# JVBSouza/descriptools

Measured on AMD Instinct MI355X. Metric: Mcells/s full descriptor chain, higher is better.
Workload: dtype f32; 1 GPU; 16384x16384 synthetic tilted-integer-fBm DEM per GPU, full chain (d8, flowacc, river mask, flowhand/HAND with fused GFI + ln(hl/H), fused slope+TI+MTI, downslope), device-resident; global_dem=16384x16384, river_threshold_cells=524288

## Files before the change

### descriptools_amd/_lib.py

```python
import ctypes as C
import os

import numpy as np

_HERE = os.path.dirname(os.path.abspath(__file__))
_SO = os.path.join(_HERE, "libdescriptools_hip.so")
_lib = None

c_f32p = C.POINTER(C.c_float)
c_f64p = C.POINTER(C.c_double)
c_u8p = C.POINTER(C.c_uint8)
c_u16p = C.POINTER(C.c_uint16)
c_i8p = C.POINTER(C.c_int8)
c_i32p = C.POINTER(C.c_int32)
c_i64p = C.POINTER(C.c_int64)
i64, f64, u32, ci = C.c_int64, C.c_double, C.c_uint32, C.c_int
vp = C.c_void_p

_SIGS = {
    "dt_last_error": (C.c_char_p, []),
    "dt_version": (C.c_char_p, []),
    "dt_device_count": (ci, []),
    "dt_set_flow_impl": (ci, [ci]),
    "dt_debug_set": (ci, [ci, ci]),
# ... 76 lines not shown
    "dt_gfi_area": (ci, [c_f32p, c_i64p, i64, f64, f64, f64, ci, c_f32p]),
    "dt_gfi": (ci, [c_f32p, c_i64p, c_i64p, i64, f64, f64, f64, c_f32p]),
    "dt_lnhlh": (ci, [c_f32p, c_i64p, i64, f64, f64, f64, c_f32p]),
    "dt_downslope": (ci, [c_f32p, c_u8p, i64, i64, f64, f64, ci, c_f32p]),
    "dt_slope_f64": (ci, [c_f64p, i64, i64, f64, c_f32p]),
    "dt_hand_f64": (ci, [c_f64p, c_i64p, i64, c_f64p]),
    "dt_downslope_f64": (ci, [c_f64p, c_u8p, i64, i64, f64, f64, ci, c_f32p]),
    "dt_gfi_f64h": (ci, [c_f64p, c_i64p, c_i64p, i64, f64, f64, f64, ci, c_f32p]),
    "dt_d8_f64": (ci, [c_f64p, i64, i64, f64, c_u8p, c_f32p]),
    "dt_confusion_multi": (ci, [c_f64p, c_i8p, i64, f64, c_f64p, ci, ci, c_i64p]),
    "dt_threshold_hist": (ci, [c_f64p, c_i8p, i64, f64, c_f64p, ci, ci, c_i64p]),
    "dt_synth_dem": (ci, [u32, i64, i64, i64, i64, i64, i64, ci, c_f32p]),
    "dt_dev_malloc": (ci, [vp, i64, C.POINTER(vp)]),
    "dt_dev_free": (ci, [vp, vp]),
    "dt_dev_h2d": (ci, [vp, vp, vp, i64]),
    "dt_dev_d2h": (ci, [vp, vp, vp, i64]),
    "dt_dev_d2h_async": (ci, [vp, vp, vp, i64]),
    "dt_dev_synth_dem": (ci, [vp, u32, i64, i64, i64, i64, i64, i64, ci, vp]),
    "dt_dev_slope_d8": (ci, [vp, vp, i64, i64, f64, vp, vp, vp]),
    "dt_dev_slope_twi": (ci, [vp, vp, vp, i64, i64, f64, f64, vp, vp, vp, vp]),
    "dt_dev_flowacc": (ci, [vp, vp, vp, i64, i64, vp]),
    "dt_dev_flowacc_weighted": (ci, [vp, vp, vp, vp, i64, i64, ci, vp]),
    "dt_dev_stream_order": (ci, [vp, vp, vp, i64, i64, vp, vp, vp]),
    "dt_dev_drainage": (ci, [vp, vp, vp, vp, i64, i64, f64, vp, vp, vp]),
    "dt_dev_upslope_length": (ci, [vp, vp, vp, i64, i64, f64, vp]),
    "dt_dev_flowpath_upslope": (ci, [vp, vp, vp, vp, i64, i64, ci, vp, vp]),
    "dt_dev_flowpath_downstream": (ci, [vp, vp, vp, vp, vp, i64, i64, ci, vp, vp]),
    "dt_dev_carve_blend": (ci, [vp, vp, vp, vp, i64, i64, f64, vp]),
    "dt_dev_flowpath_downstream_sum": (ci, [vp, vp, vp, vp, vp, i64, i64, ci, vp]),
    "dt_dev_flowpath_upslope_longest": (ci, [vp, vp, vp, vp, i64, i64, ci, vp]),
    "dt_dev_dinf_direction": (ci, [vp, vp, vp, i64, i64, f64, vp, vp]),
    "dt_dev_dinf_accumulate": (ci, [vp, vp, vp, i64, i64, ci, ci, vp]),
    "dt_dev_dinf_accumulate_info": (ci, [vp, c_i64p]),
    "dt_dev_mfd_shares": (ci, [vp, vp, vp, i64, i64, f64, ci, vp]),
    "dt_dev_mfd_accumulate": (ci, [vp, vp, vp, i64, i64, ci, ci, vp]),
    "dt_dev_mfd_accumulate_info": (ci, [vp, c_i64p]),
    "dt_dev_mfd_route": (ci, [vp, vp, vp, vp, i64, i64, ci, ci, ci] + [vp] * 4),
    "dt_dev_dinf_route": (ci, [vp, vp, vp, vp, i64, i64, ci, ci, ci] + [vp] * 4),
    "dt_dev_cost_distance": (ci, [vp, vp, vp, i64, i64, f64, ci, ci, ci, vp, vp, vp]),
    "dt_dev_wetness_suction": (ci, [vp, vp, i64, i64, f64, f64, f64, f64, vp]),
    "dt_dev_wetness_modified_area": (ci, [vp, vp, vp, i64, i64, ci, ci, vp]),
    "dt_dev_wetness_index": (ci, [vp, vp, vp, i64, i64, f64, f64, vp]),
    "dt_dev_resample": (ci, [vp, vp, ci, i64, i64, c_f64p, ci, i64, C.c_uint64, vp, i64, i64]),
    "dt_dev_morph_reconstruct": (ci, [vp, ci, ci, ci, vp, vp, vp, f64, ci, i64, i64, ci, ci, vp, vp]),
    "dt_dev_harmonic": (ci, [vp, vp, vp, vp, i64, i64, f64, ci, vp, vp]),
    "dt_dev_inundation": (ci, [vp, vp, vp, vp, i64, i64, c_f64p, ci, vp, vp, vp, ci, ci, i64, i64, vp, vp, vp, vp, vp,
                               vp]),
    "dt_dev_terrain": (ci, [vp, vp, i64, i64, f64, ci, f64, f64, f64] + [vp] * 8),
    "dt_dev_horizon": (ci, [vp, vp, i64, i64, f64, ci, ci, f64] + [vp] * 5),
    "dt_dev_focal": (ci, [vp, vp, i64, i64, f64, ci, c_i32p, ci] + [vp] * 6),
    "dt_dev_filter_extremes": (ci, [vp, vp, i64, i64, ci] + [vp] * 5),
    "dt_dev_filter_rank": (ci, [vp, vp, i64, i64, ci, c_u16p, ci, vp]),
    "dt_dev_filter_denoise": (ci, [vp, vp, i64, i64, f64, ci, f64, ci, f64, vp]),
    "dt_dev_mrvbf": (ci, [vp, vp, i64, i64, f64, f64, ci, f64, f64, c_f64p, vp, vp]),
    "dt_dev_percentile": (ci, [vp, vp, i64, i64, ci, vp, vp]),
    "dt_dev_coarsen": (ci, [vp, vp, i64, i64, f64, c_f64p, vp, vp]),
    "dt_dev_reach_catchments": (ci, [vp, vp, vp, ci, i64, i64, vp, vp, vp, i64, vp]),
    "dt_dev_reach_channels": (ci, [vp, vp, vp, i64, i64, i64, vp, vp, vp, vp, vp]),
    "dt_dev_reach_tables": (ci, [vp, vp, vp, ci, vp, i64, i64, c_f64p, ci, i64, ci, vp, vp, vp]),
    "dt_dev_inundate": (ci, [vp, vp, vp, ci, vp, i64, i64, i64, vp]),
    "dt_dev_zonal_compact": (ci, [vp, vp, ci, i64, i64, i64, vp, vp, i64, vp]),
    "dt_dev_zonal_tables": (ci, [vp, vp, vp, ci, i64, i64, i64, f64, ci, ci, f64, vp, vp, vp, vp, vp, vp]),
    "dt_dev_zonal_counts": (ci, [vp, vp, vp, ci, i64, i64, i64, c_f64p, ci, ci, f64, vp]),
    "dt_dev_zonal_paint": (ci, [vp, vp, ci, i64, vp, i64, i64, vp, vp]),
    "dt_dev_regions_label": (ci, [vp, vp, i64, i64, ci, vp, vp]),
    "dt_dev_regions_select": (ci, [vp, vp, vp, i64, i64, ci, i64, vp]),
# ... 232 lines not shown
```

### descriptools_amd/csrc/dt_capi.hip

```cpp
#include <cmath>
#include <stdarg.h>
#include <stdlib.h>

#include <sys/mman.h>
#include <atomic>
#include <chrono>
#include <mutex>
#include <system_error>
#include <thread>
#include <utility>
#include <vector>

#include "dt_common.h"
#include "dt_kernels.h"

static thread_local char g_err[512] = "";
void dt_set_error(const char *fmt, ...) {
  va_list ap;
  va_start(ap, fmt);
  vsnprintf(g_err, sizeof(g_err), fmt, ap);
  va_end(ap);
}
extern "C" const char *dt_last_error(void) { return g_err; }
extern "C" const char *dt_version(void) { return "descriptools_hip 0.1 (gfx950)"; }
// ... 1748 lines not shown
                                                      int32_t *acc32, int8_t *river, uint8_t *kind, int32_t *ref,
                                                      int32_t *nc, int32_t *nd, float *zr, int64_t *ar) {
  return dev_flowacc_finish_fh_local_w(c, win, fdr, dem, ext_perim, threshold, acc32, 0, river, kind, ref, nc, nd, zr, ar);
}
extern "C" int dt_dev_flowacc_finish_flowhand_local_w_a64(dt_ctx *c, const dt_window *win, const uint8_t *fdr,
                                                          const float *dem, const uint64_t *ext_perim,
                                                          int64_t threshold, int64_t *acc64, int8_t *river,
                                                          uint8_t *kind, int32_t *ref, int32_t *nc, int32_t *nd,
                                                          float *zr, int64_t *ar) {
  return dev_flowacc_finish_fh_local_w(c, win, fdr, dem, ext_perim, threshold, acc64, 1, river, kind, ref, nc, nd, zr, ar);
}

static int dev_flowacc_river_flowhand_local(dt_ctx *c, const uint8_t *fdr, const float *dem, const uint8_t *nod4,
                                           int64_t H, int64_t W, int64_t threshold, int32_t *acc32, int8_t *river,
                                           const DtTwiEpilogue *twi = nullptr) {
  DT_DEV(d, c, H, W);
  DT_REQUIRE((fdr && acc32 && river) || H * W == 0, "NULL raster");
  DT_REQUIRE(!twi || H * W == 0 || dt_twi_epilogue_ok(d.w, acc32, river, twi),
             "this raster does not take the TI / MTI epilogue (dt_slope_from_d8_ok): use dt_dev_slope_twi");
  const size_t need = dt_flowacc_tiled_scratch(H, W), need2 = dt_flowhand_tiled_scratch(H, W);
  void *scr, *scr2;
  d.scratch(need, need2, &scr, &scr2);
  DT_TRY(d.rc);
  DT_TRY(dt_launch_fa_local(c->stream, d.w, fdr, scr, need, acc32, 0));
  int walked = 0;
  DT_TRY(d.done(dt_launch_fa_finish_fh_local(c->stream, d.w, fdr, dem, scr, scr2, need2, nullptr, threshold, acc32, 0,
                                             river, c->status, nod4, dt_nodata4_ld(W), twi, &walked)));
  dt_scratch_claim(c, walked ? DT_OWNER_HAND_WALK : DT_OWNER_HAND, H, W, scr2);
  return DT_OK;
}
extern "C" int dt_dev_flowacc_river_flowhand_local(dt_ctx *c, const uint8_t *fdr, const float *dem, int64_t H, int64_t W,
                                                   int64_t threshold, int32_t *acc32, int8_t *river) {
  return dev_flowacc_river_flowhand_local(c, fdr, dem, nullptr, H, W, threshold, acc32, river);
}
extern "C" int dt_dev_flowacc_river_flowhand_local_m(dt_ctx *c, const uint8_t *fdr, const float *dem,
                                                     const uint8_t *nodata4, int64_t H, int64_t W, int64_t threshold,
                                                     int32_t *acc32, int8_t *river) {
  DT_REQUIRE((dem && nodata4) || H * W == 0, "dem and the nodata mask are both required");
  return dev_flowacc_river_flowhand_local(c, fdr, dem, nodata4, H, W, threshold, acc32, river);
}
extern "C" int dt_dev_flowacc_river_flowhand_local_ms(dt_ctx *c, const uint8_t *fdr, const float *dem,
                                                      const uint8_t *nodata4, int64_t H, int64_t W, int64_t threshold,
                                                      int32_t *acc32, int8_t *river, double px, double n_top,
                                                      const float *slope, float *ti, float *mti, void *marks) {
  DT_REQUIRE((dem && nodata4 && slope && ti && mti && marks) || H * W == 0, "NULL raster");
  const DtTwiEpilogue twi{slope, ti, mti, px, n_top, marks};
  return dev_flowacc_river_flowhand_local(c, fdr, dem, nodata4, H, W, threshold, acc32, river, &twi);
}
extern "C" int dt_slope_from_d8_ok(int64_t H, int64_t W) {
  return H > 0 && W > 0 && W % 64 == 0;
}
extern "C" int64_t dt_slope_marks_bytes(int64_t H, int64_t W) {
  return (H < 0 || W < 0) ? -1 : (int64_t)dt_stencil_aux_bytes(H, W);
}
extern "C" int dt_dev_slope_twi_fix(dt_ctx *c, const float *dem, const int32_t *acc32, int64_t H, int64_t W, double px,
                                    double n_top, float *slope, float *ti, float *mti, const void *marks) {
  DT_DEV(d, c, H, W);
  DT_REQUIRE((dem && acc32 && slope && ti && mti && marks) || H * W == 0, "NULL raster");
  return d.done(dt_launch_slope_twi_fix(c->stream, d.w, dem, px, slope, acc32, n_top, ti, mti, (void *)marks));
}
extern "C" int64_t dt_nodata_mask_bytes(int64_t H, int64_t W) {
  return (H < 0 || W < 0) ? -1 : (int64_t)dt_nodata4_bytes(H, W);
}
extern "C" int dt_dev_slope_d8_m(dt_ctx *c, const float *dem, int64_t H, int64_t W, double px, uint8_t *fdr,
                                 uint8_t *nodata4) {
  DT_DEV(d, c, H, W);
// ... 1997 lines not shown
```

### descriptools_amd/csrc/dt_kernels.h

```cpp
#pragma once
#include "dt_common.h"

int dt_launch_synth_dem(hipStream_t s, uint32_t seed, int O, int64_t Hg, int64_t y0, int64_t x0,
                        int64_t h, int64_t w, int nodata_pct, float *out);
int dt_launch_stencil(hipStream_t s, const DtWin &w, const float *dem, double px, float *slope,
                      uint8_t *fdr, float *slope_rad, const void *acc, int acc64, double n_top, float *ti,
                      float *mti, void *aux = nullptr, uint8_t *nod4 = nullptr, int ldm = 0);
static inline int dt_nodata4_ld(int64_t W) { return (int)((((W + 3) / 4) + 7) & ~(int64_t)7); }
static inline size_t dt_nodata4_bytes(int64_t H, int64_t W) { return (size_t)((H + 3) / 4) * (size_t)dt_nodata4_ld(W) * 2; }
struct DtStencilAux {
  uint8_t *mark;
  uint16_t *lmask;
  size_t bytes;
};
static inline DtStencilAux dt_stencil_aux_layout(int64_t ntiles, void *aux) {
  DtStencilAux a;
  DtCarver c(aux);
  a.mark = c.take<uint8_t>((size_t)ntiles);
  a.lmask = c.take<uint16_t>((size_t)ntiles * 256);
  a.bytes = c.bytes();
  return a;
}
size_t dt_stencil_aux_bytes(int64_t H, int64_t W);
int dt_launch_d8_slope(hipStream_t s, const DtWin &w, const float *dem, double px, uint8_t *fdr, float *slope,
// ... 75 lines not shown
int dt_launch_ds_walk_seed_f64(hipStream_t s, const DtWin &w, const double *dem, int64_t n, const int32_t *ys,
                               const int32_t *xs, void *rec);
int dt_launch_confusion(hipStream_t s, const double *desc, const int8_t *flood, int64_t n,
                        double nodata, const double *th_host, int nth, int under,
                        unsigned long long *counts4);
int dt_launch_threshold_hist(hipStream_t s, const double *desc, const int8_t *flood, int64_t n, double nodata,
                             const double *th_dev, int K, int under, unsigned long long *hist);
int dt_launch_i32_to_i64(hipStream_t s, const int32_t *a, int64_t n, int64_t *b);
int dt_launch_i64_to_i32(hipStream_t s, const int64_t *a, int64_t n, int32_t *b);

size_t dt_flowacc_tiled_scratch(int64_t H, int64_t W);
int dt_launch_fa_local(hipStream_t s, const DtWin &w, const uint8_t *fdr, void *scratch, size_t scratch_bytes,
                       int32_t *acc32, int rank_level);
int dt_launch_fa_summary(hipStream_t s, const DtWin &w, void *scratch, int64_t *A, int32_t *xr, uint8_t *code);
int dt_launch_fa_finish(hipStream_t s, const DtWin &w, const uint8_t *fdr, const float *dem, void *scratch,
                        const unsigned long long *ext_perim, int64_t river_thr, void *acc, int acc64,
                        int8_t *river, int *status = nullptr);
size_t dt_flowacc_weighted_scratch(int64_t H, int64_t W);
int dt_launch_flowacc_weighted(hipStream_t s, const DtWin &w, const uint8_t *fdr, const float *dem, const double *wt,
                               int frac_bits, void *scratch, size_t scratch_bytes, double *acc, int *status);
size_t dt_flowhand_tiled_scratch(int64_t H, int64_t W);
struct DtTwiEpilogue {
  const float *slope;
  float *ti, *mti;
  double px, n_top;
  void *marks;
};
int dt_launch_fa_finish_fh_local(hipStream_t s, const DtWin &w, const uint8_t *fdr, const float *dem, void *fa_scratch,
                                 void *fh_scratch, size_t fh_bytes, const unsigned long long *ext_perim,
                                 int64_t river_thr, void *acc, int acc64, int8_t *river, int *status,
                                 const uint8_t *nod4 = nullptr, int ldm = 0, const DtTwiEpilogue *twi = nullptr,
                                 int *walked = nullptr);
bool dt_twi_epilogue_ok(const DtWin &w, const void *acc, const int8_t *river, const DtTwiEpilogue *twi);
int dt_launch_fh_local(hipStream_t s, const DtWin &w, const uint8_t *fdr, const int8_t *river, void *scratch,
                       size_t scratch_bytes);
int dt_launch_fh_summary(hipStream_t s, const DtWin &w, void *scratch, const float *dem, const void *acc, int acc64,
                         uint8_t *kind, int32_t *ref, int32_t *nc, int32_t *nd, float *zr, long long *ar);
int dt_launch_fh_finish(hipStream_t s, const DtWin &w, const float *dem, const uint8_t *fdr,
                        const int8_t *river, const void *acc, int acc64, double px, void *scratch,
                        const uint8_t *res_ok, const int32_t *res_nc, const int32_t *res_nd,
                        const long long *rem_gidx, const float *rem_zr, const long long *rem_ar, float *fdist,
                        int32_t *idx32, long long *idx64, float *hand, void *a_river, float *gfi = nullptr,
                        float *lnhlh = nullptr, double n_gfi = 0.0, double b_gfi = 1.0, double size = 1.0,
                        int walked = 0);
int dt_launch_gfi_both(hipStream_t s, const float *hand, const void *a_river, const void *fac, int acc64,
                       int64_t n, double expo, double b, double size, float *gfi, float *lnhlh);
int dt_launch_unique_extremes(hipStream_t s, const float *x, int64_t n, uint32_t *work4, float *out3);
int dt_launch_minmax_scale(hipStream_t s, const float *x, int64_t n, float mn, float mx, float nodata,
                           double *out);
int dt_launch_minmax_scale_f32f64(hipStream_t s, const float *x, int64_t n, double mn, double mx, double nodata,
                                  double *out);
int dt_launch_minmax_scale_den_f32(hipStream_t s, const float *x, int64_t n, float mn, float den, float nodata,
                                   float *out);
int dt_launch_minmax_scale_den_f64(hipStream_t s, const double *x, int64_t n, double mn, double den, double nodata,
                                   double *out);
int dt_launch_minmax_scale_f16(hipStream_t s, const void *x, int64_t n, float mn, float den, float nodata, void *out);
int dt_launch_classify_f64(hipStream_t s, const double *desc, const int32_t *bin_in, int8_t *flood, int64_t n,
                           double nodata, double th, int under, int remap, uint8_t *binary, int32_t *klass,
                           unsigned long long *counts4);
int dt_launch_classify_f32(hipStream_t s, const float *desc, const int32_t *bin_in, int8_t *flood, int64_t n,
                           float nodata, float th, int under, int remap, uint8_t *binary, int32_t *klass,
                           unsigned long long *counts4);
int dt_launch_membench_copy(hipStream_t s, const float *a, float *b, int64_t n, int blocks);
int dt_launch_membench_mix(hipStream_t s, const float *r0, const float *r1, float *w0, float *w1, float *w2, int64_t n,
                           int nr, int nw, int nt);
size_t dt_rank_solve_scratch(int nranks, int64_t Pmax);
// ... 262 lines not shown
```

### descriptools_amd/csrc/dt_tiles.hip

```cpp
#include "dt_common.h"
#include "dt_kernels.h"
#include "dt_math.h"

#define TW 64
#define TH 64
#define NT (TW * TH)
#define PS (2 * TW + 2 * (TH - 2))
#define CPT (NT / 256)

#define NX_SINK 0xFFFFu
#define NX_EXIT 0xFFFEu
#define NX_REXIT 0xFFFDu
#define X_NONE 0xFFFFu

__device__ __forceinline__ int dt_slot_of(int ly, int lx) {
  if (ly == 0) return lx;
  if (ly == TH - 1) return TW + lx;
  if (lx == 0) return 2 * TW + (ly - 1);
  if (lx == TW - 1) return 2 * TW + (TH - 2) + (ly - 1);
  return -1;
}
__device__ __forceinline__ void dt_cell_of_slot(int s, int &ly, int &lx) {
  if (s < TW) { ly = 0; lx = s; }
  else if (s < 2 * TW) { ly = TH - 1; lx = s - TW; }
  else if (s < 2 * TW + (TH - 2)) { ly = s - 2 * TW + 1; lx = 0; }
  else { ly = s - 2 * TW - (TH - 2) + 1; lx = TW - 1; }
}
__device__ __forceinline__ uint32_t dt_node_of(int y, int x, int tiles_x) {
  int ty = y / TH, tx = x / TW;
  return (uint32_t)((ty * tiles_x + tx) * PS + dt_slot_of(y - ty * TH, x - tx * TW));
}

// ... 1481 lines not shown

struct TwiOut {
  const float *slope;
  float *ti, *mti;
  double n_top, lnpx2;
  uint8_t *tile_mark;
  uint32_t *lane_mask;
  int stiles_x;
};
typedef float fa_v4f __attribute__((ext_vector_type(4)));
#define FA3_WALK 0
#define FA3_TWI 0
#include "dt_fa3fh1_kernel.inc"
#undef FA3_TWI
#define FA3_TWI 1
#include "dt_fa3fh1_kernel.inc"
#undef FA3_TWI
#undef FA3_WALK
#define FA3_WALK 1
#define FA3_TWI 0
#include "dt_fa3fh1_kernel.inc"
#undef FA3_TWI
#define FA3_TWI 1
#include "dt_fa3fh1_kernel.inc"
#undef FA3_TWI
#undef FA3_WALK

__global__ __launch_bounds__(256) void k_fh_ghost_init(unsigned long long *__restrict__ nodes, uint32_t nnodes,
                                                      int64_t P) {
  int64_t i = (int64_t)blockIdx.x * 256 + threadIdx.x;
  if (i < P) nodes[nnodes + i] = fht_pack(nnodes + (uint32_t)i, 0, 0);
}

__global__ __launch_bounds__(256) void k_fh_node_jump(unsigned long long *__restrict__ state, int64_t n,
                                                      int *__restrict__ flags, int round, int hops) {
  if (flags && round > 0 && flags[round - 1] == 0) {
    if (blockIdx.x == 0 && threadIdx.x == 0) flags[round] = 0;
    return;
  }
  bool pending = false;
  for (int64_t i = (int64_t)blockIdx.x * 256 + threadIdx.x; i < n; i += (int64_t)gridDim.x * 256) {
    unsigned long long s = __hip_atomic_load(&state[i], __ATOMIC_RELAXED, __HIP_MEMORY_SCOPE_AGENT);
    bool open = false, changed = false;
    for (int h = 0; h < hops; h++) {
      const uint32_t ncf = (uint32_t)(s & 0xFFFFu);
      const uint32_t ptr = (uint32_t)(s >> 32), nd = (uint32_t)((s >> 16) & 0xFFFFu);
      if ((ncf & FHT_DONE) || ptr == (uint32_t)i) break;
      const unsigned long long t = __hip_atomic_load(&state[ptr], __ATOMIC_RELAXED, __HIP_MEMORY_SCOPE_AGENT);
      const uint32_t tptr = (uint32_t)(t >> 32), tnd = (uint32_t)((t >> 16) & 0xFFFFu);
      const uint32_t tncf = (uint32_t)(t & 0xFFFFu);
      const uint32_t nnc = ncf + (tncf & 0x7FFFu), nnd = nd + tnd;
      if (((tncf & FHT_DONE) && tptr == FHT_DEAD) || nnc + nnd > FHT_CAP) s = fht_pack(FHT_DEAD, 0, FHT_DONE);
      else s = fht_pack(tptr, nnd, nnc | (tncf & FHT_DONE));
      changed = true;
      open = !(s & (unsigned long long)FHT_DONE) && tptr != ptr;
      if (!open) break;
    }
    if (changed) __hip_atomic_store(&state[i], s, __ATOMIC_RELAXED, __HIP_MEMORY_SCOPE_AGENT);
    pending = pending || open;
  }
  if (flags && __any(pending) && (threadIdx.x & 63) == 0) flags[round] = 1;
}

template <typename AccT>
__global__ __launch_bounds__(256) void k_fh_rank_summary(DtWin w, int tiles_x, uint32_t nnodes,
                                                        const unsigned long long *__restrict__ nodes,
                                                        const float *__restrict__ dem,
                                                        const AccT *__restrict__ acc32, int64_t P,
                                                        uint8_t *__restrict__ kind, int32_t *__restrict__ ref,
                                                        int32_t *__restrict__ nc, int32_t *__restrict__ nd,
                                                        float *__restrict__ zr, long long *__restrict__ ar) {
  int64_t i = (int64_t)blockIdx.x * 256 + threadIdx.x;
  if (i >= P) return;
  int y, x;
  dt_perim_cell(w.H, w.W, i, y, x);
  const bool has_node = dt_slot_of(y % TH, x % TW) >= 0;
  unsigned long long s = has_node ? nodes[dt_node_of(y, x, tiles_x)] : fht_pack(FHT_DEAD, 0, FHT_DONE);
  uint32_t ptr = (uint32_t)(s >> 32), ncf = (uint32_t)(s & 0xFFFFu);
  uint8_t k = (uint8_t)K_DEAD;
  int32_t r = -1;
  float z = DT_NODATA;
  long long a = 0;
  if (ncf & FHT_DONE) {
    if (ptr != FHT_DEAD) {
      k = (uint8_t)K_RIVER;
      r = (int32_t)ptr;
      long long o = (long long)(ptr / (uint32_t)w.W) * w.ld + (ptr % (uint32_t)w.W);
      if (dem) z = dem[o];
      if (acc32) a = (long long)acc32[o];
    }
  } else if (ptr >= nnodes) {
    k = (uint8_t)K_REXIT;
    r = (int32_t)(ptr - nnodes);
  }
// ... 471 lines not shown

__global__ __launch_bounds__(256) void k_fh_tile3_marked(const uint8_t *__restrict__ fdr,
                                                           const float *__restrict__ dem,
                                                           const int32_t *__restrict__ acc32, DtWin w, int tiles_x,
                                                           uint32_t nnodes,
                                                           const unsigned long long *__restrict__ nodes,
                                                           const unsigned long long *__restrict__ cache,
                                                           const uint8_t *__restrict__ cache_wide, int ntiles,
                                                           double px, float *__restrict__ fdist,
                                                           int32_t *__restrict__ idx32, float *__restrict__ hand,
                                                           int32_t *__restrict__ a_river, FhGfi G) {
  __shared__ unsigned long long s_x[PS];
  __shared__ FhPay<int32_t> s_pay;
  __shared__ DtLogEntry s_tab[DT_LOGTAB_N];
  __shared__ uint8_t s_flag[256];
  const int base = (int)blockIdx.x * 256, mine = base + (int)threadIdx.x;
  const uint8_t flag = mine < ntiles ? cache_wide[mine] : (uint8_t)FH_SOLVE_LATER;
  s_flag[threadIdx.x] = flag;
  if (!__syncthreads_or(flag != FH_SOLVE_LATER)) return;
  if (G.gfi) dt_math_stage(G.tab, s_tab);
  for (int i = 0; i < 256; i++) {
    if (s_flag[i] == FH_SOLVE_LATER) continue;
    fh_tile3_tile<false, 1, int32_t, false>(s_x, s_pay, s_tab, FhSolveLds{}, nullptr, base + i, fdr, dem, acc32, w,
                                            tiles_x, nnodes, nodes, cache, s_flag[i] != 0, FhRemote{nullptr, nullptr, nullptr},
                                            px, fdist, idx32, nullptr, hand, a_river, G);
    __syncthreads();
  }
}
__global__ __launch_bounds__(256) void k_fh_mark_all(uint8_t *__restrict__ cache_wide, int ntiles) {
  const int t = (int)blockIdx.x * 256 + (int)threadIdx.x;
  if (t < ntiles && cache_wide[t] == FH_SOLVE_LATER) cache_wide[t] = 2;
}

struct FhScratch {
  unsigned long long *nodes, *cache;
  int *flags;
  uint8_t *cache_wide;
  int64_t nnodes, ntiles, P;
  int tiles_x;
  size_t bytes;
};
static FhScratch fh_layout(const DtWin &w, void *scratch) {
  FhScratch f;
  f.tiles_x = (w.W + TW - 1) / TW;
  f.ntiles = (int64_t)f.tiles_x * ((w.H + TH - 1) / TH);
  f.nnodes = f.ntiles * PS;
  f.P = dt_perim_count(w.H, w.W);
  DtCarver c(scratch);
  f.nodes = c.take<unsigned long long>((size_t)f.nnodes + (size_t)f.P);
  f.cache = c.take<unsigned long long>((size_t)f.ntiles * NT);
  f.flags = (int *)c.raw(256);
  f.cache_wide = c.take<uint8_t>((size_t)f.ntiles);
  f.bytes = c.bytes();
  return f;
}
size_t dt_flowhand_tiled_scratch(int64_t H, int64_t W) { return fh_layout(dt_full_window(H, W), nullptr).bytes; }

static int fh_local_tail(hipStream_t s, const DtWin &w, const uint8_t *fdr, const int8_t *river, const FhScratch &f,
                         bool walked = false) {
  dim3 gt((unsigned)f.ntiles), b(256);
  if (!walked)
    hipLaunchKernelGGL(k_fh_tile1, dim3(gt.x < 2048u ? gt.x : 2048u), b, 0, s, fdr, river, w, f.tiles_x,
                       (uint32_t)f.nnodes, f.nodes, f.cache, f.cache_wide, 1, (int)f.ntiles);
  hipLaunchKernelGGL(k_fh_ghost_init, dim3((unsigned)((f.P + 255) / 256)), b, 0, s, f.nodes, (uint32_t)f.nnodes, f.P);
  DT_HIP(hipMemsetAsync(f.flags, 0, 64, s));
  dim3 gj(dt_capped_grid(f.nnodes + f.P, 4096));
  for (int r = 0; r < 8; r++)
    hipLaunchKernelGGL(k_fh_node_jump, gj, b, 0, s, f.nodes, f.nnodes + f.P, f.flags, r, 3);
  return DT_OK;
}

int dt_launch_fh_local(hipStream_t s, const DtWin &w, const uint8_t *fdr, const int8_t *river, void *scratch,
                       size_t scratch_bytes) {
  if (w.H == 0 || w.W == 0) return DT_OK;
  FhScratch f = fh_layout(w, scratch);
  DT_REQUIRE(scratch_bytes >= f.bytes, "scratch too small");
  DT_REQUIRE(f.nnodes + f.P < 0x7FFFFFF0ll, "raster too large for one device tile");
  hipLaunchKernelGGL(k_fh_tile1n, dim3((unsigned)f.ntiles), dim3(256), 0, s, fdr, river, w, f.tiles_x,
                     (uint32_t)f.nnodes, f.nodes, f.cache, f.cache_wide);
  return fh_local_tail(s, w, fdr, river, f);
}

bool dt_twi_epilogue_ok(const DtWin &w, const void *acc, const int8_t *river, const DtTwiEpilogue *twi) {
  return w.W % TW == 0 && (w.ld & 3) == 0 && w.halo == 0 && w.gx0 == 0 &&
         w.gy0 == 0 && w.ld == w.W && ((uintptr_t)acc & 15) == 0 && ((uintptr_t)river & 3) == 0 && twi->marks &&
         twi->slope && twi->ti && twi->mti &&
         (((uintptr_t)twi->slope | (uintptr_t)twi->ti | (uintptr_t)twi->mti | (uintptr_t)twi->marks) & 15) == 0;
}

int dt_launch_fa_finish_fh_local(hipStream_t s, const DtWin &w, const uint8_t *fdr, const float *dem, void *fa_scratch,
                                 void *fh_scratch, size_t fh_bytes, const unsigned long long *ext_perim,
                                 int64_t river_thr, void *acc, int acc64, int8_t *river, int *status,
                                 const uint8_t *nod4, int ldm, const DtTwiEpilogue *twi, int *walked) {
  if (walked) *walked = 0;
  if (w.H == 0 || w.W == 0) return DT_OK;
  DT_REQUIRE(river != nullptr, "HAND needs the river mask");
  FaScratch f = fa_layout(w, fa_scratch);
  FhScratch h = fh_layout(w, fh_scratch);
  DT_REQUIRE(fh_bytes >= h.bytes, "scratch too small");
  DT_REQUIRE(h.nnodes + h.P < 0x7FFFFFF0ll, "raster too large for one device tile");
  dim3 gt((unsigned)f.ntiles), b(256), gn((unsigned)((f.nnodes + 255) / 256));
// ... 406 lines not shown
```

### include/descriptools_hip.h

```cpp
#ifndef DESCRIPTOOLS_HIP_H
#define DESCRIPTOOLS_HIP_H

#include <stdint.h>

#ifdef __cplusplus
extern "C" {
#endif

#define DT_OK 0
#define DT_EINVAL (-1)
#define DT_EHIP (-2)
#define DT_ENOMEM (-3)
#define DT_ENODEV (-4)

typedef struct dt_ctx dt_ctx;

typedef struct dt_window {
  int64_t H, W, ld, gy0, gx0, Hg, Wg, halo;
} dt_window;

const char *dt_last_error(void);
int dt_device_count(void);
const char *dt_version(void);
int dt_set_flow_impl(int impl);
// ... 291 lines not shown
int dt_dev_zonal_paint(dt_ctx *ctx, const void *table, int elem_bytes, int64_t n_table, const int32_t *zones,
                       int64_t rows, int64_t cols, const void *fill, void *out);
int dt_dev_cost_distance(dt_ctx *ctx, const float *friction, const int8_t *sources, int64_t rows, int64_t cols,
                         double px, int connectivity, int visit_limit, int rounds, double *cost, int64_t *indices,
                         uint8_t *backlink);
int dt_dev_wetness_suction(dt_ctx *ctx, const float *slope, int64_t rows, int64_t cols, double t, double slope_weight,
                           double slope_offset, double slope_min, float *suction);
int dt_dev_wetness_modified_area(dt_ctx *ctx, const double *area, const float *suction, int64_t rows, int64_t cols,
                                 int visit_limit, int rounds, double *modified);
int dt_dev_wetness_index(dt_ctx *ctx, const double *modified, const float *slope, int64_t rows, int64_t cols,
                         double slope_offset, double slope_min, float *swi);
int dt_dev_resample(dt_ctx *ctx, const void *src, int dtype, int64_t Hs, int64_t Ws, const double *matrix, int method,
                    int64_t nodata, uint64_t fill_bits, void *dst, int64_t Hd, int64_t Wd);
int dt_dev_morph_reconstruct(dt_ctx *ctx, int mode, int erosion, int connectivity, const float *mask,
                             const float *marker, const uint8_t *seeds, double h, int radius, int64_t rows,
                             int64_t cols, int visit_limit, int rounds, float *out, uint8_t *out8);
int dt_dev_harmonic(dt_ctx *ctx, const float *values, const int8_t *fixed, const int8_t *domain, int64_t rows,
                    int64_t cols, double tol, int max_rounds, double *out, int64_t *info);
int dt_dev_inundation(dt_ctx *ctx, const float *z, const float *manning, const float *rain, int64_t rows, int64_t cols,
                      const double *par, int boundary, const int64_t *cells, const double *times,
                      const double *discharge, int K, int T, int64_t steps0, int64_t max_steps, double *h, double *qx,
                      double *qy, double *max_depth, double *arrival, int64_t *info);
int dt_dev_regions_label(dt_ctx *ctx, const uint8_t *mask, int64_t rows, int64_t cols, int connectivity,
                         int64_t *label, int64_t *size);
int dt_dev_regions_select(dt_ctx *ctx, const uint8_t *mask, const uint8_t *seeds, int64_t rows, int64_t cols,
                          int connectivity, int64_t min_cells, uint8_t *keep);
int dt_dev_inundate_connected(dt_ctx *ctx, const int32_t *catch_, const void *hand, int hand_bytes,
                              const double *stage, const int8_t *river, int64_t rows, int64_t cols, int64_t R,
                              int connectivity, float *depth);
int dt_dev_flowacc_river(dt_ctx *ctx, const uint8_t *fdr, const float *dem, int64_t H, int64_t W,
                         int64_t threshold, int32_t *acc32, int8_t *river);
int dt_dev_flowacc_river_flowhand_local(dt_ctx *ctx, const uint8_t *fdr, const float *dem, int64_t H, int64_t W,
                                        int64_t threshold, int32_t *acc32, int8_t *river);
int64_t dt_nodata_mask_bytes(int64_t H, int64_t W);
int dt_dev_slope_d8_m(dt_ctx *ctx, const float *dem, int64_t H, int64_t W, double px, uint8_t *fdr, uint8_t *nodata4);
int dt_dev_flowacc_river_flowhand_local_m(dt_ctx *ctx, const uint8_t *fdr, const float *dem, const uint8_t *nodata4,
                                          int64_t H, int64_t W, int64_t threshold, int32_t *acc32, int8_t *river);
int dt_slope_from_d8_ok(int64_t H, int64_t W);
int64_t dt_slope_marks_bytes(int64_t H, int64_t W);
int dt_dev_slope_d8_ms(dt_ctx *ctx, const float *dem, int64_t H, int64_t W, double px, uint8_t *fdr, uint8_t *nodata4,
                       float *slope, void *marks);
int dt_dev_flowacc_river_flowhand_local_ms(dt_ctx *ctx, const uint8_t *fdr, const float *dem, const uint8_t *nodata4,
                                           int64_t H, int64_t W, int64_t threshold, int32_t *acc32, int8_t *river,
                                           double px, double n_top, const float *slope, float *ti, float *mti,
                                           void *marks);
int dt_dev_slope_twi_fix(dt_ctx *ctx, const float *dem, const int32_t *acc32, int64_t H, int64_t W, double px,
                         double n_top, float *slope, float *ti, float *mti, const void *marks);
int dt_dev_slope_d8_f64(dt_ctx *ctx, const double *dem, int64_t H, int64_t W, double px, uint8_t *fdr, float *proxy);
int dt_dev_slope_twi_f64(dt_ctx *ctx, const double *dem, const int32_t *acc32, int64_t H, int64_t W, double px,
                         double n_top, float *slope, float *slope_rad, float *ti, float *mti);
int dt_dev_downslope_f64(dt_ctx *ctx, const double *dem, const uint8_t *fdr, int64_t H, int64_t W, double px,
                         double elevation_difference, int raw, float *out);
int dt_dev_hand_gfi_f64(dt_ctx *ctx, const double *dem, const int32_t *idx32, const int32_t *acc32, int64_t H,
                        int64_t W, double px, double n_gfi, double scale_factor, double *hand, float *gfi,
                        float *lnhlh);
int dt_dev_river_mask(dt_ctx *ctx, const int32_t *acc32, int64_t N, int64_t threshold,
                      int8_t *river);
int dt_dev_flowhand(dt_ctx *ctx, const float *dem, const uint8_t *fdr, const int8_t *river,
                    const int32_t *acc32, int64_t H, int64_t W, double px, float *fdist,
                    int32_t *idx32, float *hand, int32_t *a_river);
int dt_dev_flowhand_gfi(dt_ctx *ctx, const float *dem, const uint8_t *fdr, const int8_t *river,
                        const int32_t *acc32, int64_t H, int64_t W, double px, double n_gfi, double b,
                        float *fdist, int32_t *idx32, float *hand, int32_t *a_river, float *gfi, float *lnhlh);
int dt_dev_twi(dt_ctx *ctx, const int32_t *acc32, const float *slope_rad, int64_t N, double px,
               double n_top, float *ti, float *mti);
int dt_dev_gfi(dt_ctx *ctx, const float *hand, const int32_t *a_river, int64_t N, double n_gfi,
// ... 162 lines not shown
```

Baseline: 37490 Mcells/s.

## Compact open HAND nodes into per-wave worklists for pointer jumping

```diff
diff --git a/descriptools_amd/_lib.py b/descriptools_amd/_lib.py
--- a/descriptools_amd/_lib.py
+++ b/descriptools_amd/_lib.py
@@ -132,6 +132,7 @@
     "dt_dev_dinf_direction": (ci, [vp, vp, vp, i64, i64, f64, vp, vp]),
     "dt_dev_dinf_accumulate": (ci, [vp, vp, vp, i64, i64, ci, ci, vp]),
     "dt_dev_dinf_accumulate_info": (ci, [vp, c_i64p]),
+    "dt_dev_flowhand_open_nodes": (ci, [vp, c_i64p]),
     "dt_dev_mfd_shares": (ci, [vp, vp, vp, i64, i64, f64, ci, vp]),
     "dt_dev_mfd_accumulate": (ci, [vp, vp, vp, i64, i64, ci, ci, vp]),
     "dt_dev_mfd_accumulate_info": (ci, [vp, c_i64p]),
diff --git a/descriptools_amd/csrc/dt_capi.hip b/descriptools_amd/csrc/dt_capi.hip
--- a/descriptools_amd/csrc/dt_capi.hip
+++ b/descriptools_amd/csrc/dt_capi.hip
@@ -1804,6 +1804,15 @@
 extern "C" int dt_dev_flowacc_river_flowhand_local(dt_ctx *c, const uint8_t *fdr, const float *dem, int64_t H, int64_t W,
                                                    int64_t threshold, int32_t *acc32, int8_t *river) {
   return dev_flowacc_river_flowhand_local(c, fdr, dem, nullptr, H, W, threshold, acc32, river);
+}
+extern "C" int dt_dev_flowhand_open_nodes(dt_ctx *c, int64_t *open3) {
+  DT_CTX(c);
+  DT_REQUIRE(open3 != nullptr, "open3 is NULL");
+  const DtScratchClaim *k;
+  DT_TRY(dt_scratch_claimed(c, DT_OWNER_HAND_WALK, nullptr, false,
+                            "no first phase of HAND in its walk form on this context (or another call has used the "
+                            "context's scratch since)", &k));
+  return dt_fh_open_nodes(c->stream, k->h, k->w, k->ptr, open3);
 }
 extern "C" int dt_dev_flowacc_river_flowhand_local_m(dt_ctx *c, const uint8_t *fdr, const float *dem,
                                                      const uint8_t *nodata4, int64_t H, int64_t W, int64_t threshold,
diff --git a/descriptools_amd/csrc/dt_kernels.h b/descriptools_amd/csrc/dt_kernels.h
--- a/descriptools_amd/csrc/dt_kernels.h
+++ b/descriptools_amd/csrc/dt_kernels.h
@@ -131,6 +131,7 @@
                                  const uint8_t *nod4 = nullptr, int ldm = 0, const DtTwiEpilogue *twi = nullptr,
                                  int *walked = nullptr);
 bool dt_twi_epilogue_ok(const DtWin &w, const void *acc, const int8_t *river, const DtTwiEpilogue *twi);
+int dt_fh_open_nodes(hipStream_t s, int64_t H, int64_t W, void *fh_scratch, int64_t *open3);
 int dt_launch_fh_local(hipStream_t s, const DtWin &w, const uint8_t *fdr, const int8_t *river, void *scratch,
                        size_t scratch_bytes);
 int dt_launch_fh_summary(hipStream_t s, const DtWin &w, void *scratch, const float *dem, const void *acc, int acc64,
diff --git a/descriptools_amd/csrc/dt_tiles.hip b/descriptools_amd/csrc/dt_tiles.hip
--- a/descriptools_amd/csrc/dt_tiles.hip
+++ b/descriptools_amd/csrc/dt_tiles.hip
@@ -1,3 +1,5 @@
+#include <vector>
+
 #include "dt_common.h"
 #include "dt_kernels.h"
 #include "dt_math.h"
@@ -1545,6 +1547,27 @@
   if (i < P) nodes[nnodes + i] = fht_pack(nnodes + (uint32_t)i, 0, 0);
 }
 
+__device__ __forceinline__ bool fh_node_hops(unsigned long long *__restrict__ state, uint32_t i, int hops) {
+  unsigned long long s = __hip_atomic_load(&state[i], __ATOMIC_RELAXED, __HIP_MEMORY_SCOPE_AGENT);
+  bool open = false, changed = false;
+  for (int h = 0; h < hops; h++) {
+    const uint32_t ncf = (uint32_t)(s & 0xFFFFu);
+    const uint32_t ptr = (uint32_t)(s >> 32), nd = (uint32_t)((s >> 16) & 0xFFFFu);
+    if ((ncf & FHT_DONE) || ptr == i) break;
+    const unsigned long long t = __hip_atomic_load(&state[ptr], __ATOMIC_RELAXED, __HIP_MEMORY_SCOPE_AGENT);
+    const uint32_t tptr = (uint32_t)(t >> 32), tnd = (uint32_t)((t >> 16) & 0xFFFFu);
+    const uint32_t tncf = (uint32_t)(t & 0xFFFFu);
+    const uint32_t nnc = ncf + (tncf & 0x7FFFu), nnd = nd + tnd;
+    if (((tncf & FHT_DONE) && tptr == FHT_DEAD) || nnc + nnd > FHT_CAP) s = fht_pack(FHT_DEAD, 0, FHT_DONE);
+    else s = fht_pack(tptr, nnd, nnc | (tncf & FHT_DONE));
+    changed = true;
+    open = !(s & (unsigned long long)FHT_DONE) && tptr != ptr;
+    if (!open) break;
+  }
+  if (changed) __hip_atomic_store(&state[i], s, __ATOMIC_RELAXED, __HIP_MEMORY_SCOPE_AGENT);
+  return open;
+}
+
 __global__ __launch_bounds__(256) void k_fh_node_jump(unsigned long long *__restrict__ state, int64_t n,
                                                       int *__restrict__ flags, int round, int hops) {
   if (flags && round > 0 && flags[round - 1] == 0) {
@@ -1552,27 +1575,48 @@
     return;
   }
   bool pending = false;
-  for (int64_t i = (int64_t)blockIdx.x * 256 + threadIdx.x; i < n; i += (int64_t)gridDim.x * 256) {
-    unsigned long long s = __hip_atomic_load(&state[i], __ATOMIC_RELAXED, __HIP_MEMORY_SCOPE_AGENT);
-    bool open = false, changed = false;
-    for (int h = 0; h < hops; h++) {
-      const uint32_t ncf = (uint32_t)(s & 0xFFFFu);
-      const uint32_t ptr = (uint32_t)(s >> 32), nd = (uint32_t)((s >> 16) & 0xFFFFu);
-      if ((ncf & FHT_DONE) || ptr == (uint32_t)i) break;
-      const unsigned long long t = __hip_atomic_load(&state[ptr], __ATOMIC_RELAXED, __HIP_MEMORY_SCOPE_AGENT);
-      const uint32_t tptr = (uint32_t)(t >> 32), tnd = (uint32_t)((t >> 16) & 0xFFFFu);
-      const uint32_t tncf = (uint32_t)(t & 0xFFFFu);
-      const uint32_t nnc = ncf + (tncf & 0x7FFFu), nnd = nd + tnd;
-      if (((tncf & FHT_DONE) && tptr == FHT_DEAD) || nnc + nnd > FHT_CAP) s = fht_pack(FHT_DEAD, 0, FHT_DONE);
-      else s = fht_pack(tptr, nnd, nnc | (tncf & FHT_DONE));
-      changed = true;
-      open = !(s & (unsigned long long)FHT_DONE) && tptr != ptr;
-      if (!open) break;
-    }
-    if (changed) __hip_atomic_store(&state[i], s, __ATOMIC_RELAXED, __HIP_MEMORY_SCOPE_AGENT);
-    pending = pending || open;
-  }
+  for (int64_t i = (int64_t)blockIdx.x * 256 + threadIdx.x; i < n; i += (int64_t)gridDim.x * 256)
+    pending = fh_node_hops(state, (uint32_t)i, hops) || pending;
   if (flags && __any(pending) && (threadIdx.x & 63) == 0) flags[round] = 1;
+}
+
+__device__ __forceinline__ uint32_t fh_list_append(bool open, uint32_t node, uint32_t *__restrict__ seg, uint32_t have) {
+  const unsigned long long m = __ballot(open);
+  if (open) seg[have + (uint32_t)__popcll(m & ((1ull << __lane_id()) - 1ull))] = node;
+  return have + (uint32_t)__popcll(m);
+}
+
+__global__ __launch_bounds__(256) void k_fh_node_open(unsigned long long *__restrict__ state, int64_t n, int hops,
+                                                      uint32_t *__restrict__ list, uint32_t *__restrict__ count,
+                                                      uint32_t cap) {
+  const uint32_t gw = blockIdx.x * 4u + (threadIdx.x >> 6), nw = gridDim.x * 4u, lane = threadIdx.x & 63u;
+  uint32_t *seg = list + (size_t)gw * cap;
+  uint32_t have = 0u;
+  for (int64_t b = (int64_t)gw * 64; b < n; b += (int64_t)nw * 64) {
+    const int64_t i = b + lane;
+    const bool open = i < n && fh_node_hops(state, (uint32_t)i, hops);
+    have = fh_list_append(open, (uint32_t)i, seg, have);
+  }
+  if (lane == 0u) count[gw] = have;
+}
+
+__global__ __launch_bounds__(256) void k_fh_node_list(unsigned long long *__restrict__ state,
+                                                      const uint32_t *__restrict__ in,
+                                                      const uint32_t *__restrict__ n_in, int hops,
+                                                      uint32_t *__restrict__ out, uint32_t *__restrict__ n_out,
+                                                      uint32_t cap) {
+  const uint32_t gw = blockIdx.x * 4u + (threadIdx.x >> 6), lane = threadIdx.x & 63u;
+  const uint32_t n = n_in[gw];
+  const uint32_t *seg_in = in + (size_t)gw * cap;
+  uint32_t *seg = out ? out + (size_t)gw * cap : nullptr;
+  uint32_t have = 0u;
+  for (uint32_t j = 0u; j < n; j += 64u) {
+    const uint32_t k = j + lane;
+    const uint32_t i = k < n ? seg_in[k] : 0u;
+    const bool open = k < n && fh_node_hops(state, i, hops);
+    if (out) have = fh_list_append(open, i, seg, have);
+  }
+  if (out && lane == 0u) n_out[gw] = have;
 }
 
 template <typename AccT>
@@ -2110,13 +2154,16 @@
   if (t < ntiles && cache_wide[t] == FH_SOLVE_LATER) cache_wide[t] = 2;
 }
 
+#define FH_LIST_BLOCKS 4096
+#define FH_LIST_LAUNCHES 3
 struct FhScratch {
   unsigned long long *nodes, *cache;
   int *flags;
   uint8_t *cache_wide;
+  uint32_t *list[2], *list_count[FH_LIST_LAUNCHES];
   int64_t nnodes, ntiles, P;
   int tiles_x;
-  size_t bytes;
+  size_t bytes, list_bytes;
 };
 static FhScratch fh_layout(const DtWin &w, void *scratch) {
   FhScratch f;
@@ -2130,21 +2177,57 @@
   f.flags = (int *)c.raw(256);
   f.cache_wide = c.take<uint8_t>((size_t)f.ntiles);
   f.bytes = c.bytes();
+  const size_t list_blocks = dt_capped_grid(f.nnodes, FH_LIST_BLOCKS);
+  DtCarver lc(f.cache);
+  for (int k = 0; k < FH_LIST_LAUNCHES; k++) f.list_count[k] = lc.take<uint32_t>(list_blocks * 4);
+  for (int k = 0; k < 2; k++) f.list[k] = lc.take<uint32_t>((size_t)f.nnodes + list_blocks * 256);
+  f.list_bytes = lc.bytes();
   return f;
 }
 size_t dt_flowhand_tiled_scratch(int64_t H, int64_t W) { return fh_layout(dt_full_window(H, W), nullptr).bytes; }
 
+#define FH_HOPS_FIRST 3
+#define FH_HOPS_LIST 17
 static int fh_local_tail(hipStream_t s, const DtWin &w, const uint8_t *fdr, const int8_t *river, const FhScratch &f,
                          bool walked = false) {
   dim3 gt((unsigned)f.ntiles), b(256);
-  if (!walked)
-    hipLaunchKernelGGL(k_fh_tile1, dim3(gt.x < 2048u ? gt.x : 2048u), b, 0, s, fdr, river, w, f.tiles_x,
-                       (uint32_t)f.nnodes, f.nodes, f.cache, f.cache_wide, 1, (int)f.ntiles);
+  if (walked) {
+    static_assert(FH_LIST_LAUNCHES == 3 && (FH_HOPS_FIRST + 1) * (FH_HOPS_LIST + 1) * (FH_HOPS_LIST + 1) *
+                                                   (FH_HOPS_LIST + 1) >= (int)FHT_CAP + 1,
+                  "the launch plan must cover FHT_CAP moves");
+    DT_REQUIRE(f.list_bytes <= (size_t)f.ntiles * NT * sizeof(unsigned long long), "node lists larger than the word cache");
+    const dim3 gl(dt_capped_grid(f.nnodes, FH_LIST_BLOCKS));
+    const int64_t per_pass = (int64_t)gl.x * 256;
+    const uint32_t cap = (uint32_t)((f.nnodes + per_pass - 1) / per_pass) * 64u;
+    hipLaunchKernelGGL(k_fh_node_open, gl, b, 0, s, f.nodes, f.nnodes, FH_HOPS_FIRST, f.list[0], f.list_count[0], cap);
+    for (int k = 0; k < FH_LIST_LAUNCHES; k++) {
+      const bool last = k + 1 == FH_LIST_LAUNCHES;
+      hipLaunchKernelGGL(k_fh_node_list, gl, b, 0, s, f.nodes, (const uint32_t *)f.list[k & 1],
+                         (const uint32_t *)f.list_count[k], FH_HOPS_LIST,
+                         last ? (uint32_t *)nullptr : f.list[(k + 1) & 1],
+                         last ? (uint32_t *)nullptr : f.list_count[k + 1], cap);
+    }
+    return DT_OK;
+  }
+  hipLaunchKernelGGL(k_fh_tile1, dim3(gt.x < 2048u ? gt.x : 2048u), b, 0, s, fdr, river, w, f.tiles_x,
+                     (uint32_t)f.nnodes, f.nodes, f.cache, f.cache_wide, 1, (int)f.ntiles);
   hipLaunchKernelGGL(k_fh_ghost_init, dim3((unsigned)((f.P + 255) / 256)), b, 0, s, f.nodes, (uint32_t)f.nnodes, f.P);
   DT_HIP(hipMemsetAsync(f.flags, 0, 64, s));
   dim3 gj(dt_capped_grid(f.nnodes + f.P, 4096));
   for (int r = 0; r < 8; r++)
     hipLaunchKernelGGL(k_fh_node_jump, gj, b, 0, s, f.nodes, f.nnodes + f.P, f.flags, r, 3);
+  return DT_OK;
+}
+
+int dt_fh_open_nodes(hipStream_t s, int64_t H, int64_t W, void *fh_scratch, int64_t *open3) {
+  const FhScratch f = fh_layout(dt_full_window(H, W), fh_scratch);
+  std::vector<uint32_t> len((size_t)dt_capped_grid(f.nnodes, FH_LIST_BLOCKS) * 4);
+  for (int k = 0; k < FH_LIST_LAUNCHES; k++) {
+    DT_HIP(hipMemcpyAsync(len.data(), f.list_count[k], len.size() * sizeof(uint32_t), hipMemcpyDeviceToHost, s));
+    DT_HIP(hipStreamSynchronize(s));
+    open3[k] = 0;
+    for (uint32_t v : len) open3[k] += (int64_t)v;
+  }
   return DT_OK;
 }
 
diff --git a/include/descriptools_hip.h b/include/descriptools_hip.h
--- a/include/descriptools_hip.h
+++ b/include/descriptools_hip.h
@@ -347,6 +347,7 @@
                          int64_t threshold, int32_t *acc32, int8_t *river);
 int dt_dev_flowacc_river_flowhand_local(dt_ctx *ctx, const uint8_t *fdr, const float *dem, int64_t H, int64_t W,
                                         int64_t threshold, int32_t *acc32, int8_t *river);
+int dt_dev_flowhand_open_nodes(dt_ctx *ctx, int64_t *open3);
 int64_t dt_nodata_mask_bytes(int64_t H, int64_t W);
 int dt_dev_slope_d8_m(dt_ctx *ctx, const float *dem, int64_t H, int64_t W, double px, uint8_t *fdr, uint8_t *nodata4);
 int dt_dev_flowacc_river_flowhand_local_m(dt_ctx *ctx, const uint8_t *fdr, const float *dem, const uint8_t *nodata4,
```

New measurement: 37430 Mcells/s. About the same (-0.1%).
